# Sicco123/YieldFactorModels.jl

Hardware: AMD Instinct MI355X
Metric: Kalman loglik evals/sec (DNS, T=600, N=30) (higher is better)
Workload: dtype f64

## Files before the change

### yieldfactormodels.jl_amd/csrc/yfm_fixedz.hpp

```cpp
#pragma once
#pragma clang fp contract(off)
#include "yfm_device.hpp"

namespace yfm {

template <int M>
__device__ __forceinline__ double collapsed_cov(const double (&R)[M][M], const double (&Pm)[M][M], LDLT<M>& f,
                                                double (&Pf)[M][M]) {
  double S[M][M];
#pragma unroll
  for (int i = 0; i < M; ++i)
#pragma unroll
    for (int j = 0; j <= i; ++j) S[i][j] = Pm[i][j] + R[i][j];
  const double det = f.factor(S);
#pragma unroll
  for (int j = 0; j < M; ++j) {
    double xj[M];
#pragma unroll
    for (int i = 0; i < M; ++i) xj[i] = R[i][j];
    f.solve(xj);
#pragma unroll
    for (int i = 0; i <= j; ++i) {
      double s = 0.0;
#pragma unroll
// ... 433 lines not shown
    last_q = upd ? q : __builtin_nan("");
    if (acc) {
      if (STEADY && was_frozen) {
        count_frozen(det);
      } else {
        ld.mul(det);
        neg = neg || (det < 0.0);
      }
      sumq += last_q;
    }
  }

  __device__ __forceinline__ void record(int t, int b, int my_steps, int rec_len, double* __restrict__ rec_beta,
                                         double* __restrict__ rec_P) const {
    const int slot = t - max(0, my_steps - rec_len);
    if (t < my_steps && slot >= 0) {
      const size_t o = (size_t)b * (size_t)rec_len + slot;
#pragma unroll
      for (int i = 0; i < M; ++i) rec_beta[o * M + i] = beta[i];
      if (rec_P) {
#pragma unroll
        for (int j = 0; j < M; ++j)
#pragma unroll
          for (int i = 0; i < M; ++i) rec_P[o * M * M + j * M + i] = Pm[i][j];
      }
    }
  }

  __device__ __forceinline__ double loglik(int nobs, unsigned int* __restrict__ flags) const {
    double ll;
    if (!init_ok) {
      ll = __builtin_nan("");
      atomicAdd(&flags[0], 1u);
    } else {
      const int nterms = max(nobs - 2, 0);
      if (nterms == 0) {
        ll = 0.0;
      } else {
        const double per_term = (double)(N - M) * log(sigma2) + logdetG + (double)N * kLog2Pi;
        double lf = 0.0;
        if constexpr (STEADY) lf = fzlog + (nfz == 0 ? 0.0 : (double)nfz * log(fabs(fzdet)));
        ll = -0.5 * ((double)nterms * per_term + (ld.log_value() + lf) + sumq);
      }
      const bool fneg = STEADY && nfz != 0 && fzdet < 0.0;
      if (neg || fneg || !isfinite(ll)) {
        ll = -__builtin_inf();
        atomicAdd(&flags[1], 1u);
      }
    }
    return ll;
  }
};

}
```

### yieldfactormodels.jl_amd/csrc/yfm_internal.hpp

```cpp
#pragma once
#include "yfm_flags.hpp"
#include <hip/hip_runtime.h>

#include "../../include/yfm.h"

namespace yfm {

struct DevBuf {
  void* p = nullptr;
  size_t cap = 0;
  DevBuf() = default;
  DevBuf(const DevBuf&) = delete;
  DevBuf& operator=(const DevBuf&) = delete;
  ~DevBuf() {
    if (p) (void)hipFree(p);
  }
  hipError_t ensure(size_t bytes) {
    if (bytes <= cap) return hipSuccess;
    if (p) (void)hipFree(p);
    p = nullptr;
    cap = 0;
    hipError_t e = hipMalloc(&p, bytes);
    if (e == hipSuccess) cap = bytes;
    return e;
  }
};

struct LaunchArgs {
  const double* theta;
  int P, B, space;
  const double* panel;
  const double* raw;
  int T, N, np, ldp;
  const double* mats;
  const int* T_use;
  double* out;
  unsigned int* flags;
  unsigned int* flags_next = nullptr;
  double* rec_beta;
  double* rec_P;
  double* scratch;
  int horizon = 0;
  int rec_len = 0;
  int* defer_list = nullptr;
  int* defer_count = nullptr;
  hipStream_t stream;
};

int fixedz_np_for(int N);
hipError_t launch_fixedz(int kind, const LaunchArgs& a);
bool dns_split_supported(int np);
hipError_t launch_dns_split(const LaunchArgs& a);
size_t fixedz_scratch_bytes(int kind, int B);
int group_max_n(int kind);
int group_lanes_for(int kind, int N);
hipError_t launch_fixedz_group(int kind, const LaunchArgs& a);
size_t fixedz_dd_scratch_bytes(int kind, int B);
hipError_t launch_fixedz_dd(int kind, const LaunchArgs& a, double* rec);
int grad_max_n();
hipError_t launch_dns_grad(const LaunchArgs& a, const double* ll, double* grad_out);
int tvl_lanes_for(int B, int N, int share = 1);
int tvl_max_n();
size_t tvl_scratch_bytes(int B);
constexpr int kTvlGaps = 8;
constexpr int kTvlPowGaps = 16;
struct TvlGaps {
  int K = 0;
  bool exact = false;
  const double* d = nullptr;
  const int* idx = nullptr;
  int Kp = 0;
  double step = 0.0;
  const double* e = nullptr;
  const int* pidx = nullptr;
};
hipError_t launch_tvl(const LaunchArgs& a, const TvlGaps& g, int lanes);
constexpr int kRecSigma = 0, kRecDelta = 1, kRecPhi = 5, kRecQ = 21, kRecBeta = 31, kRecP = 35, kRecOk = 45;
constexpr int kRecLen = 48;
size_t tvl_dd_scratch_bytes(int B);
size_t tvl_dd_colsum_bytes(int T);
int tvl_dd_lanes_for(int B, int N, int want, int share = 1);
hipError_t launch_tvl_dd_colsum(const double* Y, int N, int T, double* colsum, hipStream_t s);
hipError_t launch_tvl_dd_init(const LaunchArgs& a, double* rec_dd);
hipError_t launch_tvl_dd(const LaunchArgs& a, const double* rec_dd, const double* colsum, const TvlGaps& g, int lanes);
struct PredictArgs {
  int kind, M, L, N, P, B, T;
  int ncol;
  int horizon;
  const double* theta;
  const double* mats;
  const int* T_use;
  const double* rec;
  int rec_len;
  const unsigned char* init_bad;
  double* preds;
  double* factors;
  double* states;
  double* load1;
  double* load2;
  hipStream_t stream;
};
hipError_t launch_init_bad(const double* ll, int B, unsigned char* bad, hipStream_t s);
hipError_t launch_predict_emit(const PredictArgs& a);
hipError_t launch_forecast_emit(const PredictArgs& a);
hipError_t launch_loss_array(const PredictArgs& a, const double* Y, int T1, int passes, unsigned int* flags);
// ... 12 lines not shown
```

### yieldfactormodels.jl_amd/csrc/yfm_kernels.hip

```cpp
#include "yfm_fixedz.hpp"

namespace yfm {

constexpr int kBlock = 256;
constexpr int kTC = 64;
constexpr bool kMfma4 = true;
constexpr bool kZBasis = true;

__global__ void prep_panel_kernel(const double* __restrict__ Y, int N, int T, int np, int ldp,
                                  double* __restrict__ out) {
  const int t = blockIdx.x * blockDim.x + threadIdx.x;
  if (t >= T) return;
  const double* y = Y + (size_t)t * N;
  double* o = out + (size_t)t * ldp;
  double s1 = 0.0, yy = 0.0;
  bool nan = false;
  for (int i = 0; i < N; ++i) {
    const double v = y[i];
    nan = nan || (v != v);
    s1 += v;
    yy = fma(v, v, yy);
  }
  const double ybar = s1 / (double)N;
  double tt = 0.0;
// ... 140 lines not shown
    }
    const double piv = col[k];
    ok = ok && (piv != 0.0);
    const double rp = 1.0 / piv;
#pragma unroll
    for (int i = k + 1; i < S; ++i) {
      const double l = col[i] * rp;
#pragma unroll
      for (int s = sk; s < NS; ++s) a[s][i] = fma(-l, a[s][k], a[s][i]);
    }
  }
  double x[S];
#pragma unroll
  for (int k = S - 1; k >= 0; --k) {
    const double rp = role_bcast_from<R>(k % R, 1.0 / a[k / R][k]);
    double s = role_bcast_from<R>(S % R, a[S / R][k]);
#pragma unroll
    for (int j = k + 1; j < S; ++j) s = role_bcast_from<R>(j % R, fma(-a[j / R][k], x[j], s));
    x[k] = s * rp;
  }
  if (role != 0) return;
  int q = 0;
#pragma unroll
  for (int i = 0; i < M; ++i) rec[(size_t)(q++) * B + b] = beta[i];
#pragma unroll
  for (int r = 0; r < S; ++r) rec[(size_t)(q++) * B + b] = x[r];
  rec[(size_t)q * B + b] = ok ? 1.0 : 0.0;
}


template <int NP, int NZ>
__device__ __forceinline__ void dot_zt(const double* __restrict__ col, const double (&Zc)[NZ][NP], double (&zt)[NZ]) {
  double a[NZ][2];
#pragma unroll
  for (int cz = 0; cz < NZ; ++cz) {
    a[cz][0] = 0.0;
    a[cz][1] = 0.0;
  }
#pragma unroll
  for (int i = 0; i < NP; i += 2) {
    const double2 y2 = *reinterpret_cast<const double2*>(col + i);
#pragma unroll
    for (int cz = 0; cz < NZ; ++cz) {
      a[cz][0] = fma(Zc[cz][i], y2.x, a[cz][0]);
      a[cz][1] = fma(Zc[cz][i + 1], y2.y, a[cz][1]);
    }
  }
#pragma unroll
  for (int cz = 0; cz < NZ; ++cz) zt[cz] = a[cz][0] + a[cz][1];
}

typedef double yfm_double4 __attribute__((ext_vector_type(4)));

template <int NP, int M, int LEAD, bool RECORD, bool STEADY_ = false, bool SPLIT_FORM = false>
__global__ __launch_bounds__(kBlock, 1) void fixedz_loglik_kernel(
    const double* __restrict__ theta, int P, int B, int space, const double* __restrict__ panel, int T, int N,
    const double* __restrict__ mats, const int* __restrict__ T_use, double* __restrict__ out,
    unsigned int* __restrict__ flags, double* __restrict__ rec_beta, double* __restrict__ rec_P, int horizon,
    int rec_len, int* __restrict__ defer_list, int* __restrict__ defer_count, const double* __restrict__ init_rec,
    unsigned int* __restrict__ flags_next, int steady) {
  constexpr int LDP = NP + 4;
  constexpr int TC = (M == 3) ? kTC : 32;
  constexpr bool USE_MFMA_ = (M - 1 == 2 || M - 1 == 4) && (NP <= 32);
  constexpr bool STEADY = STEADY_ && !RECORD && (M == 3 || M == 5) && USE_MFMA_;
  constexpr bool SPLIT_INIT = (M == 5);
  constexpr int CH = TC * LDP;
  constexpr int PER = (CH + kBlock - 1) / kBlock;
  constexpr int NZ = M - 1;
  constexpr bool USE_MFMA = (NZ == 2 || NZ == 4) && (NP <= 32);
  constexpr int NK = (NP + 3) / 4;
  constexpr int NRT = 64 * NZ / 16;
  constexpr int RGN = 4;
  constexpr int RGN4 = (NZ == 2) ? NRT : 8;
  constexpr int TB = 16;
  constexpr bool ZB = USE_MFMA && kMfma4 && kZBasis && LEAD == 2;
  constexpr int RPC = ZB ? LEAD : NZ;
  constexpr int NRTA = 64 * RPC / 16;
  constexpr int SS = 64 * NZ + 2;
  constexpr int SCR = USE_MFMA ? ((TB * SS > 32 * RPC * (4 * NK + 1)) ? TB * SS : 32 * RPC * (4 * NK + 1)) : 2;
  static_assert(NZ == 2 * LEAD, "loading columns come in (S, C) pairs per gamma");
  static_assert(NP % 2 == 0, "double2 panel reads");
  static_assert(TC % TB == 0, "MFMA blocks tile the panel chunk");
  __shared__ __attribute__((aligned(16))) double sh[2][CH];
  __shared__ __attribute__((aligned(16))) double scratch[kBlock / 64][SCR];
  __shared__ int s_nobs_max;
  __shared__ double s_rm[ZB ? NP : 1];

  if (flags_next && blockIdx.x == 0 && threadIdx.x < kFlagsPerBank) flags_next[threadIdx.x] = 0u;
  const int tid = threadIdx.x;
  const int lane = tid & 63;
  const int wave = tid >> 6;
  const int b = blockIdx.x * kBlock + tid;
  const bool live = b < B;
  const int bb = live ? b : (B - 1);
  const int nobs = T_use ? T_use[bb] : T;

  auto load_into = [&](double* dst, int c) {
    const size_t base = (size_t)c * CH;
    const size_t lim = (size_t)T * LDP;
#pragma unroll
    for (int r = 0; r < PER; ++r) {
      const int e = r * kBlock + tid;
      const size_t g = base + e;
      dst[r] = (e < CH && g < lim) ? panel[g] : 0.0;
    }
  };
  auto store_from = [&](const double* src, double* buf) {
#pragma unroll
    for (int r = 0; r < PER; ++r) {
      const int e = r * kBlock + tid;
      if (e < CH) buf[e] = src[r];
    }
  };
  constexpr bool EARLY = M == 3 && NP <= 32;
  double pre0[EARLY ? PER : 1], pre1[EARLY ? PER : 1];
  if constexpr (EARLY) {
    load_into(pre0, 0);
    load_into(pre1, 1);
  }

  if (tid == 0) s_nobs_max = 0;
  if constexpr (ZB) {
    for (int i = tid; i < NP; i += kBlock) s_rm[i] = (i < N) ? 1.0 / mats[i] : 0.0;
// ... 12 lines not shown
      const double* src = theta + (size_t)w0 * kP;
      double* thl = scratch[wave];
      double v[kP];
#pragma unroll
      for (int r = 0; r < kP; ++r) {
        const int e = r * 64 + lane;
        v[r] = (e < n) ? src[e] : 0.0;
      }
#pragma unroll
      for (int r = 0; r < kP; ++r) thl[r * 64 + lane] = v[r];
      __builtin_amdgcn_s_waitcnt(0xc07f);
      __builtin_amdgcn_wave_barrier();
      th_row = thl + (bb - w0) * kP;
    }
  }
  Params<M, LEAD> p;
  decode_params<M, LEAD>(th_row, space, p);
  __builtin_amdgcn_s_waitcnt(0xc07f);
  __builtin_amdgcn_wave_barrier();

  double Zc[NZ][NP];
#pragma unroll
  for (int l = 0; l < LEAD; ++l) {
    const double lam = 1e-2 + exp(p.gam[l]);
#pragma unroll
    for (int i = 0; i < NP; ++i) {
      const double tau = lam * mats[max(min(i, N - 1), 0)];
      const double z = exp(-tau);
      const double s = (1.0 - z) / tau;
      Zc[2 * l][i] = (i < N) ? s : 0.0;
      Zc[2 * l + 1][i] = (i < N) ? s - z : 0.0;
    }
  }
  double G[M][M];
  G[0][0] = (double)N;
#pragma unroll
  for (int c = 0; c < NZ; ++c) {
    double s = 0.0;
#pragma unroll
    for (int i = 0; i < NP; ++i) s += Zc[c][i];
    G[0][c + 1] = s;
    G[c + 1][0] = s;
#pragma unroll
    for (int d = c; d < NZ; ++d) {
      double g = 0.0;
#pragma unroll
      for (int i = 0; i < NP; ++i) g = fma(Zc[c][i], Zc[d][i], g);
      G[c + 1][d + 1] = g;
      G[d + 1][c + 1] = g;
    }
  }

  constexpr bool SIGMA = USE_MFMA && !ZB && !(kMfma4 && NZ == 4);
  constexpr bool IL = SIGMA && NRT == 2 * RGN && NK == 2 * RGN;
  constexpr bool IL5 = ZB && NK == NRTA;
  auto sigma = [](int i) { return SIGMA ? 4 * (i & 3) + (i >> 2) : i; };
  double Af[USE_MFMA ? NRTA : 1][USE_MFMA ? NK : 1];
  double rlam[LEAD];
#pragma unroll
  for (int l = 0; l < LEAD; ++l) rlam[l] = 1.0 / (1e-2 + exp(p.gam[l]));
  if constexpr (USE_MFMA) {
    constexpr int ZS = 4 * NK + 1;
    constexpr int HT = NRTA / 2;
    static_assert(32 * RPC * ZS <= SCR, "staging fits the scratch");
    double* st = scratch[wave];
#pragma unroll
    for (int h = 0; h < 2; ++h) {
      if ((lane >> 5) == h) {
        const int cl = lane & 31;
        if constexpr (ZB) {
#pragma unroll
          for (int l = 0; l < LEAD; ++l) {
            const double lam = 1e-2 + exp(p.gam[l]);
#pragma unroll
            for (int m = 0; m < ZS; ++m) {
              const double e = 1.0 - exp(-(lam * mats[max(min(m, N - 1), 0)]));
              st[(cl * RPC + l) * ZS + m] = (m < N) ? e : 0.0;
            }
          }
        } else {
#pragma unroll
          for (int c = 0; c < NZ; ++c)
#pragma unroll
            for (int m = 0; m < ZS; ++m) st[(cl * NZ + c) * ZS + m] = (m < NP) ? Zc[c][m] : 0.0;
        }
      }
      __builtin_amdgcn_s_waitcnt(0xc07f);
      __builtin_amdgcn_wave_barrier();
#pragma unroll
      for (int r = h * HT; r < (h + 1) * HT; ++r) {
        const int pr = 16 * r + sigma(lane & 15) - h * 32 * RPC;
#pragma unroll
        for (int kk = 0; kk < NK; ++kk) Af[r][kk] = st[pr * ZS + 4 * kk + (lane >> 4)];
      }
      __builtin_amdgcn_s_waitcnt(0xc07f);
      __builtin_amdgcn_wave_barrier();
    }
  }

  FixedZFilter<M, LEAD, RECORD, STEADY, SPLIT_FORM> f;
  f.p = p;
  f.steady_ok = steady != 0;
  f.setup(G, N, !SPLIT_INIT);
  if constexpr (SPLIT_INIT) {
    int q = 0;
#pragma unroll
    for (int i = 0; i < M; ++i) f.beta[i] = init_rec[(size_t)(q++) * B + bb];
#pragma unroll
    for (int i = 0; i < M; ++i)
#pragma unroll
      for (int j = i; j < M; ++j) {
        const double v = init_rec[(size_t)(q++) * B + bb];
        f.Pm[i][j] = v;
        f.Pm[j][i] = v;
      }
    f.init_ok = init_rec[(size_t)q * B + bb] != 0.0;
  }
  const bool defer = live && !f.collapsed;
  if (defer) defer_list[atomicAdd(defer_count, 1)] = b;

  int wmin = live ? my_data : 0x7fffffff;
#pragma unroll
  for (int off = 32; off >= 1; off >>= 1) wmin = min(wmin, __shfl_xor(wmin, off));
  const int wave_min_data = __builtin_amdgcn_readfirstlane(wmin);
  const bool wave_all_collapsed = true;

  __syncthreads();
  const int nsteps = max(s_nobs_max, 0);

  double pre[PER];
  auto load_chunk = [&](int c) { load_into(pre, c); };
  auto store_chunk = [&](double* buf) { store_from(pre, buf); };
  if (nsteps > 0) {
    if constexpr (EARLY) {
      store_from(pre0, sh[0]);
      store_from(pre1, sh[1]);
    } else {
// ... 106 lines not shown
            const int m = 4 * kk + (lane >> 4);
            const double y = (m < NP) ? cb[(2 * sp + ((lane & 3) >> 1)) * LDP + m] : 0.0;
            bv[kk] = (lane & 1) ? y * s_rm[m < NP ? m : 0] : y;
          }
#pragma unroll
          for (int r0 = 0; r0 < NRTA; r0 += NRTA) {
            double acc[NRTA];
#pragma unroll
            for (int r = 0; r < NRTA; ++r) acc[r] = 0.0;
#pragma unroll
            for (int kk = 0; kk < NK; ++kk)
#pragma unroll
              for (int r = 0; r < NRTA; ++r)
                acc[r] = __builtin_amdgcn_mfma_f64_4x4x4f64(Af[r][kk], bv[kk], acc[r], 0, 0, 0);
#pragma unroll
            for (int r = 0; r < NRTA; ++r)
              scr[(2 * sp + ((lane & 3) >> 1)) * SS + 2 * (16 * r + 4 * ((lane >> 2) & 3) + (lane >> 4)) + (lane & 1)] =
                  acc[r];
          }
        }
      } else if constexpr (kMfma4 && NZ == 4) {
#pragma unroll
        for (int s = 0; s < TB / 4; ++s) {
          double bv[NK];
#pragma unroll
          for (int kk = 0; kk < NK; ++kk) {
            const int m = 4 * kk + (lane >> 4);
            bv[kk] = (m < NP) ? cb[(4 * s + (lane & 3)) * LDP + m] : 0.0;
          }
#pragma unroll
          for (int r0 = 0; r0 < NRT; r0 += RGN4) {
            double acc[RGN4];
#pragma unroll
            for (int r = 0; r < RGN4; ++r) acc[r] = 0.0;
#pragma unroll
            for (int kk = 0; kk < NK; ++kk)
#pragma unroll
              for (int r = 0; r < RGN4; ++r)
                acc[r] = __builtin_amdgcn_mfma_f64_4x4x4f64(Af[r0 + r][kk], bv[kk], acc[r], 0, 0, 0);
#pragma unroll
            for (int r = 0; r < RGN4; ++r)
              scr[(4 * s + (lane & 3)) * SS + 16 * (r0 + r) + 4 * ((lane >> 2) & 3) + (lane >> 4)] = acc[r];
          }
        }
      } else {
        double bvk[NK];
#pragma unroll
        for (int kk = 0; kk < NK; ++kk) {
          const int m = 4 * kk + (lane >> 4);
          bvk[kk] = (m < NP) ? cb[(lane & 15) * LDP + m] : 0.0;
        }
        if constexpr (IL) {
          constexpr int H = RGN / 2;
          yfm_double4 a1[RGN], a2[H], a3[H];
#pragma unroll
          for (int r = 0; r < RGN; ++r) a1[r] = yfm_double4{0.0, 0.0, 0.0, 0.0};
#pragma unroll
          for (int r = 0; r < H; ++r) a2[r] = a3[r] = yfm_double4{0.0, 0.0, 0.0, 0.0};
#pragma unroll
          for (int kk = 0; kk < NK; ++kk)
#pragma unroll
            for (int r = 0; r < RGN; ++r)
              a1[r] = __builtin_amdgcn_mfma_f64_16x16x4f64(Af[r][kk], bvk[kk], a1[r], 0, 0, 0);
#pragma unroll
          for (int kk = 0; kk < NK; ++kk) {
#pragma unroll
            for (int r = 0; r < H; ++r)
              a2[r] = __builtin_amdgcn_mfma_f64_16x16x4f64(Af[RGN + r][kk], bvk[kk], a2[r], 0, 0, 0);
            const int r1 = kk >> 1, h = kk & 1;
            double* d = scr + (lane & 15) * SS + 16 * r1 + 4 * (lane >> 4) + 2 * h;
            *reinterpret_cast<double2*>(d) = make_double2(a1[r1][2 * h], a1[r1][2 * h + 1]);
          }
#pragma unroll
          for (int kk = 0; kk < NK; ++kk) {
#pragma unroll
            for (int r = 0; r < H; ++r)
              a3[r] = __builtin_amdgcn_mfma_f64_16x16x4f64(Af[RGN + H + r][kk], bvk[kk], a3[r], 0, 0, 0);
            if (kk & 1) {
              const int r2 = kk >> 2, h = (kk >> 1) & 1;
              double* d = scr + (lane & 15) * SS + 16 * (RGN + r2) + 4 * (lane >> 4) + 2 * h;
              *reinterpret_cast<double2*>(d) = make_double2(a2[r2][2 * h], a2[r2][2 * h + 1]);
            }
          }
          __builtin_amdgcn_sched_group_barrier(0x008, RGN * NK, 0);
#pragma unroll
          for (int kk = 0; kk < NK; ++kk) {
            __builtin_amdgcn_sched_group_barrier(0x008, H, 0);
            __builtin_amdgcn_sched_group_barrier(0x200, 1, 0);
          }
#pragma unroll
          for (int kk = 0; kk < NK; ++kk) {
            __builtin_amdgcn_sched_group_barrier(0x008, H, 0);
            if (kk & 1) __builtin_amdgcn_sched_group_barrier(0x200, 1, 0);
          }
#pragma unroll
          for (int r = 0; r < H; ++r) store_tile(scr, RGN + H + r, a3[r]);
        } else {
#pragma unroll
        for (int r0 = 0; r0 < NRT; r0 += RGN) {
          yfm_double4 acc[RGN];
#pragma unroll
          for (int r = 0; r < RGN; ++r) acc[r] = yfm_double4{0.0, 0.0, 0.0, 0.0};
#pragma unroll
          for (int kk = 0; kk < NK; ++kk)
#pragma unroll
            for (int r = 0; r < RGN; ++r)
              acc[r] = __builtin_amdgcn_mfma_f64_16x16x4f64(Af[r0 + r][kk], bvk[kk], acc[r], 0, 0, 0);
#pragma unroll
          for (int r = 0; r < RGN; ++r) store_tile(scr, r0 + r, acc[r]);
        }
        }
      }
      __builtin_amdgcn_s_waitcnt(0xc07f);
      __builtin_amdgcn_wave_barrier();
      const int tend = min(TB, nsteps - t0);
      bool blk_steady = false;
      if constexpr (STEADY) {
        if (__all(f.wave_frozen) && t0 >= 1 && t0 + tend <= wave_min_data) {
          const bool col_nan = (lane < tend) && (col_flag != 0.0);
          blk_steady = !__any(col_nan);
        }
      }
      auto read_z = [&](int tt, double (&z)[NZ]) {
        const double* sp = scr + tt * SS + NZ * lane;
#pragma unroll
        for (int j = 0; j < NZ; j += 2) {
          const double2 v = *reinterpret_cast<const double2*>(sp + j);
          if constexpr (ZB) {
            z[j] = rlam[j / 2] * v.y;
            z[j + 1] = z[j] + v.x;
          } else {
            z[j] = v.x;
            z[j + 1] = v.y;
          }
        }
      };
      double zc[NZ];
      read_z(0, zc);
      double2 yb = *reinterpret_cast<const double2*>(cb + NP);
      double2 meta = *reinterpret_cast<const double2*>(cb + NP + 2);
      double zn[NZ];
      double2 ybn, metan;
      auto half = [&](int tt, const double (&zc_)[NZ], double2 yb_, double2 meta_, double (&zn_)[NZ], double2& ybn_,
                      double2& metan_) {
        const int t = t0 + tt;
        const int tn = min(tt + 1, TB - 1);
        read_z(tn, zn_);
        ybn_ = *reinterpret_cast<const double2*>(cb + tn * LDP + NP);
        metan_ = *reinterpret_cast<const double2*>(cb + tn * LDP + NP + 2);
        do_step(t, zc_, yb_, meta_);
        record(t);
        if ((t + 1) % TC == 0) rot_t = t;
      };
      auto shalf = [&](int tt, const double (&zc_)[NZ], double2 yb_, double (&zn_)[NZ], double2& ybn_) {
        const int tn = min(tt + 1, TB - 1);
        read_z(tn, zn_);
        ybn_ = *reinterpret_cast<const double2*>(cb + tn * LDP + NP);
        f.steady_step(zc_, yb_);
        if ((t0 + tt + 1) % TC == 0) rot_t = t0 + tt;
      };
      if constexpr (STEADY) {
        if (blk_steady) {
          if (tend == TB) {
            double zq[2][NZ];
            double2 ybq[2];
#pragma unroll
            for (int j = 0; j < NZ; ++j) zq[0][j] = zc[j];
            ybq[0] = yb;
#pragma unroll
            for (int u = 0; u < TB; ++u) {
              const int cur = u & 1, nx = cur ^ 1;
              const int tn = min(u + 1, TB - 1);
              read_z(tn, zq[nx]);
              ybq[nx] = *reinterpret_cast<const double2*>(cb + tn * LDP + NP);
              f.steady_step(zq[cur], ybq[cur]);
            }
            rot_t = ((t0 + TB) % TC == 0) ? t0 + TB - 1 : -1;
          } else {
            int tt = 0;
            for (; tt + 1 < tend; tt += 2) {
              shalf(tt, zc, yb, zn, ybn);
              shalf(tt + 1, zn, ybn, zc, yb);
            }
            if (tt < tend) shalf(tt, zc, yb, zn, ybn);
          }
          steady_steps += tend;
          f.count_steady(tend);
        }
      }
      if (!blk_steady) {
        int tt = 0;
        bool rest_steady = false;
        for (; tt + 1 < tend; tt += 2) {
          half(tt, zc, yb, meta, zn, ybn, metan);
          half(tt + 1, zn, ybn, metan, zc, yb, meta);
          if constexpr (STEADY) {
            if (tt == TB / 2 - 2) f.prepare_bound();
            {
              const int r0 = tt + 2;
              if (r0 >= TB / 2 && r0 < tend && t0 + tend <= wave_min_data) {
                const bool nan_rest = (lane >= r0) && (lane < tend) && (col_flag != 0.0);
                if (!__any(nan_rest)) {
                  f.wave_freeze(live && !defer && f.init_ok && t0 + tend <= my_steps);
                  if (f.wave_frozen) {
                    rest_steady = true;
                    tt = r0;
                    break;
                  }
                }
              }
            }
          }
        }
        if constexpr (STEADY) {
          if (rest_steady) {
            const int n = tend - tt;
            for (; tt + 1 < tend; tt += 2) {
              shalf(tt, zc, yb, zn, ybn);
              shalf(tt + 1, zn, ybn, zc, yb);
            }
            if (tt < tend) shalf(tt, zc, yb, zn, ybn);
            steady_steps += n;
            f.count_steady(n);
          }
        }
        if (!rest_steady) {
          if (tt < tend) half(tt, zc, yb, meta, zn, ybn, metan);
          if constexpr (STEADY) f.wave_freeze(live && !defer && f.init_ok && t0 + tend <= my_steps);
        }
      }
      __builtin_amdgcn_s_waitcnt(0xc07f);
      __builtin_amdgcn_wave_barrier();
    }
    if (rot_t >= 0) rotate(rot_t);
    if constexpr (STEADY) {
      if (lane == 0 && steady_steps) atomicAdd(&flags[4], steady_steps);
    }
  } else {
    double zc[NZ];
    double2 yb_c = make_double2(0.0, 0.0), meta_c = make_double2(0.0, 0.0);
    if (nsteps > 0) {
      const double* c0 = col_of(0);
      dot_zt<NP, NZ>(c0, Zc, zc);
      yb_c = *reinterpret_cast<const double2*>(c0 + NP);
      meta_c = *reinterpret_cast<const double2*>(c0 + NP + 2);
    }
    double zn[NZ];
    double2 yb_n, meta_n;
    auto half = [&](int t, const double (&zc_)[NZ], double2 yb_, double2 meta_, double (&zn_)[NZ], double2& ybn_,
                    double2& metan_) {
      const double* cn = col_of(t + 1);
      dot_zt<NP, NZ>(cn, Zc, zn_);
      ybn_ = *reinterpret_cast<const double2*>(cn + NP);
      metan_ = *reinterpret_cast<const double2*>(cn + NP + 2);
      do_step(t, zc_, yb_, meta_);
      record(t);
      rotate(t);
    };
    int t = 0;
    for (; t + 1 < nsteps; t += 2) {
      half(t, zc, yb_c, meta_c, zn, yb_n, meta_n);
      half(t + 1, zn, yb_n, meta_n, zc, yb_c, meta_c);
    }
    if (t < nsteps) half(t, zc, yb_c, meta_c, zn, yb_n, meta_n);
  }

  if (!live || defer) return;
  const double ll = f.loglik(nobs, flags);
  out[b] = ll;
}

}

#include "yfm_internal.hpp"

#include <cstdlib>

namespace yfm {

static int steady_enabled() {
  const char* e = std::getenv("YFM_DNS_STEADY");
  return (e && e[0] == '0') ? 0 : 1;
}

static int gns5_steady_enabled() {
  const char* e = std::getenv("YFM_GNS5_STEADY");
  return (e && e[0] == '1') ? 1 : 0;
}

static int split_form_enabled() {
  const char* e = std::getenv("YFM_FZ_SPLIT_FORM");
  return (e && e[0] == '1') ? 1 : 0;
}

static int gns5_init_lanes() {
  const char* e = std::getenv("YFM_GNS5_INIT_LANES");
  return (e && e[0] == '1' && e[1] == 0) ? 1 : 2;
}

template <int NP, int M, int LEAD>
static hipError_t launch_fixedz_np(const LaunchArgs& a) {
  const int grid = (a.B + kBlock - 1) / kBlock;
  if constexpr (M == 5) {
    if (!a.scratch) return hipErrorInvalidValue;
    const int ir = gns5_init_lanes();
    if (ir == 1) {
      hipLaunchKernelGGL((fixedz_init_kernel<M, LEAD>), dim3(grid), dim3(kBlock), 0, a.stream, a.theta, a.P, a.B,
                         a.space, a.scratch, a.flags_next);
    } else {
      const int gi = (int)(((size_t)a.B * 2 + kBlock - 1) / kBlock);
      hipLaunchKernelGGL((fixedz_init_coop_kernel<M, LEAD, 2>), dim3(gi), dim3(kBlock), 0, a.stream, a.theta, a.P, a.B,
                         a.space, a.scratch, a.flags_next);
    }
  }
  if (a.rec_beta) {
    hipLaunchKernelGGL((fixedz_loglik_kernel<NP, M, LEAD, true>), dim3(grid), dim3(kBlock), 0, a.stream, a.theta, a.P,
                       a.B, a.space, a.panel, a.T, a.N, a.mats, a.T_use, a.out, a.flags, a.rec_beta, a.rec_P,
                       a.horizon, a.rec_len, a.defer_list, a.defer_count, a.scratch, M == 5 ? nullptr : a.flags_next, 0);
  } else {
    constexpr bool kSteady = (M == 3 || M == 5) && (NP <= 32);
    constexpr int kSteadyMinT = 80;
    const bool on = steady_enabled() && a.T >= kSteadyMinT && (M != 5 || gns5_steady_enabled());
    auto* k = (kSteady && on) ? &fixedz_loglik_kernel<NP, M, LEAD, false, kSteady>
                              : &fixedz_loglik_kernel<NP, M, LEAD, false, false>;
    constexpr bool kSplitForm = (M == 5) && (NP == 30 || NP == 48);
    if constexpr (kSplitForm) {
      if (split_form_enabled()) k = &fixedz_loglik_kernel<NP, M, LEAD, false, false, true>;
    }
    hipLaunchKernelGGL(k, dim3(grid), dim3(kBlock), 0, a.stream, a.theta, a.P, a.B, a.space, a.panel, a.T, a.N,
                       a.mats, a.T_use, a.out, a.flags, nullptr, nullptr, 0, 0, a.defer_list, a.defer_count,
                       a.scratch, M == 5 ? nullptr : a.flags_next, 1);
  }
  return hipGetLastError();
}

size_t fixedz_scratch_bytes(int kind, int B) {
  return kind == 2 ? sizeof(double) * (size_t)fz_rec_len<5>() * (size_t)(B > 0 ? B : 1) : 0;
}

int fixedz_np_for(int N) {
  if (N <= 8) return 8;
  if (N <= 16) return 16;
  if (N <= 24) return 24;
  if (N <= 30) return 30;
  if (N <= 32) return 32;
  if (N <= 48) return 48;
  if (N <= 64) return 64;
  return -1;
}

hipError_t launch_fixedz(int kind, const LaunchArgs& a) {
  if (kind == 0 && dns_split_supported(a.np)) {
    const char* e = std::getenv("YFM_DNS_SPLIT");
    if (e && e[0] == '1') return launch_dns_split(a);
  }
  if (kind == 0) {
    switch (a.np) {
      case 8: return launch_fixedz_np<8, 3, 1>(a);
      case 16: return launch_fixedz_np<16, 3, 1>(a);
      case 24: return launch_fixedz_np<24, 3, 1>(a);
      case 30: return launch_fixedz_np<30, 3, 1>(a);
      case 32: return launch_fixedz_np<32, 3, 1>(a);
      case 48: return launch_fixedz_np<48, 3, 1>(a);
      case 64: return launch_fixedz_np<64, 3, 1>(a);
    }
  } else if (kind == 2) {
    switch (a.np) {
      case 8: return launch_fixedz_np<8, 5, 2>(a);
      case 16: return launch_fixedz_np<16, 5, 2>(a);
      case 24: return launch_fixedz_np<24, 5, 2>(a);
      case 30: return launch_fixedz_np<30, 5, 2>(a);
      case 32: return launch_fixedz_np<32, 5, 2>(a);
      case 48: return launch_fixedz_np<48, 5, 2>(a);
      case 64: return launch_fixedz_np<64, 5, 2>(a);
    }
  }
  return hipErrorInvalidValue;
}

hipError_t launch_prep_panel(const double* Y, int N, int T, int np, int ldp, double* out, hipStream_t s) {
  hipLaunchKernelGGL(prep_panel_kernel, dim3((T + 63) / 64), dim3(64), 0, s, Y, N, T, np, ldp, out);
// ... 5 lines not shown
```

### yieldfactormodels.jl_amd/csrc/yfm_split.hip

```cpp
#include "yfm_fixedz.hpp"
#include "yfm_internal.hpp"

#include <cstdlib>
#include <type_traits>

namespace yfm {

namespace {

constexpr int kSplitBlock = 512;
constexpr int kSplitPairs = 4;
constexpr int kSTC = 32;
constexpr int kSTB = 16;
constexpr int kRec = 13;

}

template <int NP, bool RECORD>
__global__ __launch_bounds__(kSplitBlock, 1) void dns_split_kernel(
    const double* __restrict__ theta, int P, int B, int space, const double* __restrict__ panel, int T, int N,
    const double* __restrict__ mats, const int* __restrict__ T_use, double* __restrict__ out,
    unsigned int* __restrict__ flags, double* __restrict__ rec_beta, double* __restrict__ rec_P, int horizon,
    int rec_len, int* __restrict__ defer_list, int* __restrict__ defer_count, int interleave,
    unsigned int* __restrict__ flags_next) {
  constexpr int M = 3, LEAD = 1, NZ = 2;
  if (flags_next && blockIdx.x == 0 && threadIdx.x < kFlagsPerBank) flags_next[threadIdx.x] = 0u;
  constexpr int LDP = NP + 4;
  constexpr int CH = kSTC * LDP;
  constexpr int PER = (CH + kSplitBlock - 1) / kSplitBlock;
  constexpr int NK = (NP + 3) / 4;
  constexpr int NRT = 64 * NZ / 16;
  constexpr int SS = 64 * NZ + 2;
  constexpr int SCR = kSTB * SS;
  static_assert(NP <= 32 && NP % 2 == 0, "MFMA fragments and double2 panel reads");
  __shared__ __attribute__((aligned(16))) double sh[2][CH];
  __shared__ __attribute__((aligned(16))) double scratch[kSplitPairs][SCR];
  __shared__ double ring[2][kSplitPairs][kRec][64];
  __shared__ int s_nobs_max;

  const int tid = threadIdx.x;
  const int lane = tid & 63;
  const int wave = tid >> 6;
  const bool cov = interleave ? !(wave & 1) : wave < kSplitPairs;
  const int pair = interleave ? (wave >> 1) : (wave & (kSplitPairs - 1));
  const int b = blockIdx.x * (kSplitPairs * 64) + pair * 64 + lane;
  const bool live = b < B;
  const int bb = live ? b : (B - 1);
  const int nobs = T_use ? T_use[bb] : T;

  if (tid == 0) s_nobs_max = 0;
  __syncthreads();
  const int my_steps = horizon > 0 ? nobs + horizon : nobs - 1;
  const int my_data = horizon > 0 ? nobs : nobs - 1;
  atomicMax(&s_nobs_max, live ? my_steps : 0);

  auto role = [&](auto is_cov) {
    constexpr bool COV = decltype(is_cov)::value;
  FixedZFilter<M, LEAD, RECORD> f;
  decode_params<M, LEAD>(theta + (size_t)bb * P, space, f.p);
  const double lam = 1e-2 + exp(f.p.gam[0]);
  auto loading = [&](int i, double& s, double& c) {
    if (i < N) {
      const double tau = lam * mats[i];
      const double z = exp(-tau);
      s = (1.0 - z) / tau;
      c = s - z;
    } else {
      s = 0.0;
      c = 0.0;
    }
  };
  double G[M][M];
  double gs[NZ] = {0.0, 0.0}, gg[3] = {0.0, 0.0, 0.0};
  auto acc_gram = [&](double s, double c) {
    gs[0] += s;
    gs[1] += c;
    gg[0] = fma(s, s, gg[0]);
    gg[1] = fma(s, c, gg[1]);
    gg[2] = fma(c, c, gg[2]);
  };
#pragma unroll
  for (int i = 0; i < NP; ++i) {
    double zs, zc;
    loading(i, zs, zc);
    acc_gram(zs, zc);
  }
  G[0][0] = (double)N;
  G[0][1] = G[1][0] = gs[0];
  G[0][2] = G[2][0] = gs[1];
  G[1][1] = gg[0];
  G[1][2] = G[2][1] = gg[1];
  G[2][2] = gg[2];
  f.setup(G, N, true);
  const bool defer = live && !f.collapsed;
  if constexpr (!COV) {
    if (defer) defer_list[atomicAdd(defer_count, 1)] = b;
  }
  double Af[COV ? 1 : NRT][COV ? 1 : NK];
  if constexpr (!COV) {
    constexpr int ZS = 4 * NK + 1;
    constexpr int QT = NRT / 4;
    static_assert(16 * NZ * ZS <= SCR, "staging fits the scratch");
    double* st = scratch[pair];
#pragma unroll
    for (int qu = 0; qu < 4; ++qu) {
      if ((lane >> 4) == qu) {
        const int cl = lane & 15;
#pragma unroll
        for (int m = 0; m < ZS; ++m) {
          double zs, zc;
          loading(m < NP ? m : NP, zs, zc);
          st[(cl * NZ + 0) * ZS + m] = zs;
          st[(cl * NZ + 1) * ZS + m] = zc;
        }
      }
      __builtin_amdgcn_s_waitcnt(0xc07f);
      __builtin_amdgcn_wave_barrier();
#pragma unroll
      for (int r = qu * QT; r < (qu + 1) * QT; ++r) {
        const int pr = 16 * r + (lane & 15) - qu * 16 * NZ;
#pragma unroll
        for (int kk = 0; kk < NK; ++kk) Af[r][kk] = st[pr * ZS + 4 * kk + (lane >> 4)];
      }
      __builtin_amdgcn_s_waitcnt(0xc07f);
      __builtin_amdgcn_wave_barrier();
    }
  }

  int wmin = live ? my_data : 0x7fffffff;
#pragma unroll
  for (int off = 32; off >= 1; off >>= 1) wmin = min(wmin, __shfl_xor(wmin, off));
  const int wave_min_data = __builtin_amdgcn_readfirstlane(wmin);

  __syncthreads();
  const int nsteps = max(s_nobs_max, 0);

  double pre[PER];
  auto load_chunk = [&](int c) {
    const size_t base = (size_t)c * CH;
    const size_t lim = (size_t)T * LDP;
#pragma unroll
    for (int r = 0; r < PER; ++r) {
      const int e = r * kSplitBlock + tid;
      const size_t g = base + e;
      pre[r] = (e < CH && g < lim) ? panel[g] : 0.0;
    }
  };
  auto store_chunk = [&](double* buf) {
#pragma unroll
    for (int r = 0; r < PER; ++r) {
      const int e = r * kSplitBlock + tid;
      if (e < CH) buf[e] = pre[r];
    }
  };
  if (nsteps > 0) {
    load_chunk(0);
    store_chunk(sh[0]);
    load_chunk(1);
    store_chunk(sh[1]);
    __syncthreads();
    load_chunk(2);
  }
  auto col_of = [&](int t) -> const double* { return sh[(t / kSTC) & 1] + (t % kSTC) * LDP; };
  auto lds_barrier = [] {
// ... 45 lines not shown
#pragma unroll
            for (int j = i; j < M; ++j) Pf[i][j] = f.Pm[i][j];
          propagate_cov_f<M>(phi, f.p.Q, Pf, f.Pm);
        }
        if constexpr (RECORD) {
          const int rs = t - max(0, my_steps - rec_len);
          if (rec_P && live && !defer && act && rs >= 0) {
            const size_t o = (size_t)b * (size_t)rec_len + rs;
#pragma unroll
            for (int j = 0; j < M; ++j)
#pragma unroll
              for (int i = 0; i < M; ++i) rec_P[o * M * M + j * M + i] = f.Pm[i][j];
          }
        }
      }
      end_iteration(k);
    }
  } else {
  double* scr = scratch[pair];
  for (int k = 0; k <= nsteps; ++k) {
    if (k >= 1) {
      const int t = k - 1;
      const int tt = t % kSTB;
      if (tt == 0) {
        const double* cb = col_of(t);
        double bvk[NK];
#pragma unroll
        for (int kk = 0; kk < NK; ++kk) {
          const int m = 4 * kk + (lane >> 4);
          bvk[kk] = (m < NP) ? cb[(lane & 15) * LDP + m] : 0.0;
        }
        typedef double d4 __attribute__((ext_vector_type(4)));
        constexpr int RG = NRT / 4;
#pragma unroll
        for (int r0 = 0; r0 < NRT; r0 += RG) {
          d4 acc[RG];
#pragma unroll
          for (int r = 0; r < RG; ++r) acc[r] = d4{0.0, 0.0, 0.0, 0.0};
#pragma unroll
          for (int kk = 0; kk < NK; ++kk)
#pragma unroll
            for (int r = 0; r < RG; ++r)
              acc[r] = __builtin_amdgcn_mfma_f64_16x16x4f64(Af[r0 + r][kk], bvk[kk], acc[r], 0, 0, 0);
#pragma unroll
          for (int r = 0; r < RG; ++r)
#pragma unroll
            for (int q4 = 0; q4 < 4; ++q4) scr[(lane & 15) * SS + 16 * (r0 + r) + (lane >> 4) + 4 * q4] = acc[r][q4];
        }
        __builtin_amdgcn_s_waitcnt(0xc07f);
        __builtin_amdgcn_wave_barrier();
      }
      const double* cb = col_of(t);
      const double2 z2 = *reinterpret_cast<const double2*>(scr + tt * SS + NZ * lane);
      const double zc[NZ] = {z2.x, z2.y};
      const double2 yb = *reinterpret_cast<const double2*>(cb + NP);
      const double2 meta = *reinterpret_cast<const double2*>(cb + NP + 2);
      const bool fast = (t >= 1) && (meta.x == 0.0) && (t < wave_min_data);
      const bool act = t < my_steps;
      if (fast || (act && meta.x == 0.0 && t < my_data)) {
        const double* slot = &ring[t & 1][pair][0][lane];
        LDLT<M> fl;
        fl.L[1][0] = slot[0 * 64];
        fl.L[2][0] = slot[1 * 64];
        fl.L[2][1] = slot[2 * 64];
        fl.rd[0] = slot[3 * 64];
        fl.rd[1] = slot[4 * 64];
        fl.rd[2] = slot[5 * 64];
        double Pm[M][M];
        Pm[0][0] = slot[6 * 64];
        Pm[0][1] = Pm[1][0] = slot[7 * 64];
        Pm[0][2] = Pm[2][0] = slot[8 * 64];
        Pm[1][1] = slot[9 * 64];
        Pm[1][2] = Pm[2][1] = slot[10 * 64];
        Pm[2][2] = slot[11 * 64];
        const double det = slot[12 * 64];
        double bf[M], q;
        collapsed_mean<M>(zc, yb.x, yb.y, f.R, f.rsig2, f.beta, Pm, fl, bf, q);
        if (fast) {
          if (!RECORD || det != 0.0) propagate_mean_f<M>(phi, f.p.delta, bf, f.beta);
          f.last_det = det;
          f.last_q = q;
          f.ld.mul(det);
          f.sumq += q;
          f.neg = f.neg || (det < 0.0);
        } else {
          const bool upd = det != 0.0;
          if (upd) propagate_mean_f<M>(phi, f.p.delta, bf, f.beta);
          f.last_det = det;
          f.last_q = upd ? q : __builtin_nan("");
          if (t >= 1) {
            f.ld.mul(det);
            f.sumq += f.last_q;
            f.neg = f.neg || (det < 0.0);
          }
        }
      } else if (act) {
        double bf[M];
#pragma unroll
        for (int i = 0; i < M; ++i) bf[i] = f.beta[i];
        propagate_mean_f<M>(phi, f.p.delta, bf, f.beta);
        if (t >= 1) {
          f.ld.mul(f.last_det);
          f.sumq += f.last_q;
          f.neg = f.neg || (f.last_det < 0.0);
        }
      }
      if constexpr (RECORD) {
        const int rs = t - max(0, my_steps - rec_len);
        if (live && !defer && act && rs >= 0) {
          const size_t o = (size_t)b * (size_t)rec_len + rs;
#pragma unroll
          for (int i = 0; i < M; ++i) rec_beta[o * M + i] = f.beta[i];
        }
      }
      if (tt == kSTB - 1) {
        __builtin_amdgcn_s_waitcnt(0xc07f);
        __builtin_amdgcn_wave_barrier();
      }
    }
    end_iteration(k);
  }

  if (!live || defer) return;
  out[b] = f.loglik(nobs, flags);
  }

  };
  if (cov)
    role(std::true_type{});
  else
    role(std::false_type{});
}

namespace {

template <int NP>
hipError_t launch_split_np(const LaunchArgs& a) {
  const int interleave = 0;
  const int grid = (a.B + kSplitPairs * 64 - 1) / (kSplitPairs * 64);
  if (a.rec_beta) {
    hipLaunchKernelGGL((dns_split_kernel<NP, true>), dim3(grid), dim3(kSplitBlock), 0, a.stream, a.theta, a.P, a.B,
                       a.space, a.panel, a.T, a.N, a.mats, a.T_use, a.out, a.flags, a.rec_beta, a.rec_P, a.horizon,
                       a.rec_len, a.defer_list, a.defer_count, interleave, a.flags_next);
  } else {
    hipLaunchKernelGGL((dns_split_kernel<NP, false>), dim3(grid), dim3(kSplitBlock), 0, a.stream, a.theta, a.P, a.B,
                       a.space, a.panel, a.T, a.N, a.mats, a.T_use, a.out, a.flags, nullptr, nullptr, 0, 0,
                       a.defer_list, a.defer_count, interleave, a.flags_next);
  }
  return hipGetLastError();
}

}

bool dns_split_supported(int np) { return np == 8 || np == 16 || np == 24 || np == 30 || np == 32; }

hipError_t launch_dns_split(const LaunchArgs& a) {
  switch (a.np) {
    case 8: return launch_split_np<8>(a);
    case 16: return launch_split_np<16>(a);
    case 24: return launch_split_np<24>(a);
    case 30: return launch_split_np<30>(a);
    case 32: return launch_split_np<32>(a);
  }
  return hipErrorInvalidValue;
}

}
```

Baseline: 375.7 million.

## Trim MFMA K-dimension for N=30 DNS by folding loading column into difference form

For NP=30, M=3, the loading matrix is rewritten as differences against the last observed column, so the projection needs only 28 K-slots (7 MFMA k-steps instead of 8). The leftover column at slot 28 is added back per step with an FMA using the raw panel value. Interleaved scheduling barriers and tile stores are generalized to odd NK. This cuts MFMA work in the projection at the cost of an extra load and FMA per step, and it relies on the panel's padding and column layout being arranged so that the difference form reproduces the original sums.

```diff
diff --git a/yieldfactormodels.jl_amd/csrc/yfm_fixedz.hpp b/yieldfactormodels.jl_amd/csrc/yfm_fixedz.hpp
--- a/yieldfactormodels.jl_amd/csrc/yfm_fixedz.hpp
+++ b/yieldfactormodels.jl_amd/csrc/yfm_fixedz.hpp
@@ -509,4 +509,19 @@
   }
 };
 
-}
+constexpr int kTrimNP = 30;
+constexpr int kTrimSlot = 28;
+constexpr bool ktrim_applies(int NP, int M) { return NP == kTrimNP && M == 3; }
+constexpr int ktrim_nk(int NP, bool trim) { return trim ? (kTrimSlot / 4) : (NP + 3) / 4; }
+
+__device__ __forceinline__ double ktrim_diff(double z, double z_last, int i, int N) {
+  return (i < N - 1) ? z - z_last : 0.0;
+}
+
+template <int NZ>
+__device__ __forceinline__ void ktrim_leftover(const double (&zd)[NZ], const double (&zx)[NZ + 1], double (&z)[NZ]) {
+#pragma unroll
+  for (int c = 0; c < NZ; ++c) z[c] = fma(zd[c], zx[NZ], zx[c]);
+}
+
+}
diff --git a/yieldfactormodels.jl_amd/csrc/yfm_internal.hpp b/yieldfactormodels.jl_amd/csrc/yfm_internal.hpp
--- a/yieldfactormodels.jl_amd/csrc/yfm_internal.hpp
+++ b/yieldfactormodels.jl_amd/csrc/yfm_internal.hpp
@@ -51,6 +51,7 @@
 hipError_t launch_fixedz(int kind, const LaunchArgs& a);
 bool dns_split_supported(int np);
 hipError_t launch_dns_split(const LaunchArgs& a);
+int ktrim_enabled();
 size_t fixedz_scratch_bytes(int kind, int B);
 int group_max_n(int kind);
 int group_lanes_for(int kind, int N);
diff --git a/yieldfactormodels.jl_amd/csrc/yfm_kernels.hip b/yieldfactormodels.jl_amd/csrc/yfm_kernels.hip
--- a/yieldfactormodels.jl_amd/csrc/yfm_kernels.hip
+++ b/yieldfactormodels.jl_amd/csrc/yfm_kernels.hip
@@ -216,8 +216,8 @@
 
 typedef double yfm_double4 __attribute__((ext_vector_type(4)));
 
-template <int NP, int M, int LEAD, bool RECORD, bool STEADY_ = false, bool SPLIT_FORM = false>
-__global__ __launch_bounds__(kBlock, 1) void fixedz_loglik_kernel(
+template <int NP, int M, int LEAD, bool RECORD, bool STEADY_, bool SPLIT_FORM, bool KTRIM_>
+__device__ __forceinline__ void fixedz_loglik_body(
     const double* __restrict__ theta, int P, int B, int space, const double* __restrict__ panel, int T, int N,
     const double* __restrict__ mats, const int* __restrict__ T_use, double* __restrict__ out,
     unsigned int* __restrict__ flags, double* __restrict__ rec_beta, double* __restrict__ rec_P, int horizon,
@@ -232,7 +232,8 @@
   constexpr int PER = (CH + kBlock - 1) / kBlock;
   constexpr int NZ = M - 1;
   constexpr bool USE_MFMA = (NZ == 2 || NZ == 4) && (NP <= 32);
-  constexpr int NK = (NP + 3) / 4;
+  constexpr bool KTRIM = KTRIM_ && USE_MFMA && ktrim_applies(NP, M);
+  constexpr int NK = ktrim_nk(NP, KTRIM);
   constexpr int NRT = 64 * NZ / 16;
   constexpr int RGN = 4;
   constexpr int RGN4 = (NZ == 2) ? NRT : 8;
@@ -351,10 +352,21 @@
   }
 
   constexpr bool SIGMA = USE_MFMA && !ZB && !(kMfma4 && NZ == 4);
-  constexpr bool IL = SIGMA && NRT == 2 * RGN && NK == 2 * RGN;
+  constexpr bool IL = SIGMA && NRT == 2 * RGN && (NK == 2 * RGN || NK == 2 * RGN - 1);
   constexpr bool IL5 = ZB && NK == NRTA;
   auto sigma = [](int i) { return SIGMA ? 4 * (i & 3) + (i >> 2) : i; };
   double Af[USE_MFMA ? NRTA : 1][USE_MFMA ? NK : 1];
+  double z_last[KTRIM ? NZ : 1], zd28[KTRIM ? NZ : 1];
+  if constexpr (KTRIM) {
+#pragma unroll
+    for (int c = 0; c < NZ; ++c) {
+      double zl = 0.0;
+#pragma unroll
+      for (int i = 0; i < NP; ++i) zl = (i == N - 1) ? Zc[c][i] : zl;
+      z_last[c] = zl;
+      zd28[c] = ktrim_diff(Zc[c][kTrimSlot], zl, kTrimSlot, N);
+    }
+  }
   double rlam[LEAD];
 #pragma unroll
   for (int l = 0; l < LEAD; ++l) rlam[l] = 1.0 / (1e-2 + exp(p.gam[l]));
@@ -381,7 +393,12 @@
 #pragma unroll
           for (int c = 0; c < NZ; ++c)
 #pragma unroll
-            for (int m = 0; m < ZS; ++m) st[(cl * NZ + c) * ZS + m] = (m < NP) ? Zc[c][m] : 0.0;
+            for (int m = 0; m < ZS; ++m) {
+              if constexpr (KTRIM)
+                st[(cl * NZ + c) * ZS + m] = ktrim_diff(Zc[c][m], z_last[c], m, N);
+              else
+                st[(cl * NZ + c) * ZS + m] = (m < NP) ? Zc[c][m] : 0.0;
+            }
         }
       }
       __builtin_amdgcn_s_waitcnt(0xc07f);
@@ -594,6 +611,9 @@
         }
         if constexpr (IL) {
           constexpr int H = RGN / 2;
+          constexpr int NS1 = 2 * RGN, NS2 = 2 * H;
+          auto last1 = [](int kk) { return kk == NK - 1 ? NS1 : kk + 1; };
+          auto at2 = [](int s) { return 2 * s + 1 < NK - 1 ? 2 * s + 1 : NK - 1; };
           yfm_double4 a1[RGN], a2[H], a3[H];
 #pragma unroll
           for (int r = 0; r < RGN; ++r) a1[r] = yfm_double4{0.0, 0.0, 0.0, 0.0};
@@ -609,31 +629,40 @@
 #pragma unroll
             for (int r = 0; r < H; ++r)
               a2[r] = __builtin_amdgcn_mfma_f64_16x16x4f64(Af[RGN + r][kk], bvk[kk], a2[r], 0, 0, 0);
-            const int r1 = kk >> 1, h = kk & 1;
-            double* d = scr + (lane & 15) * SS + 16 * r1 + 4 * (lane >> 4) + 2 * h;
-            *reinterpret_cast<double2*>(d) = make_double2(a1[r1][2 * h], a1[r1][2 * h + 1]);
+#pragma unroll
+            for (int s = kk; s < last1(kk); ++s) {
+              const int r1 = s >> 1, h = s & 1;
+              double* d = scr + (lane & 15) * SS + 16 * r1 + 4 * (lane >> 4) + 2 * h;
+              *reinterpret_cast<double2*>(d) = make_double2(a1[r1][2 * h], a1[r1][2 * h + 1]);
+            }
           }
 #pragma unroll
           for (int kk = 0; kk < NK; ++kk) {
 #pragma unroll
             for (int r = 0; r < H; ++r)
               a3[r] = __builtin_amdgcn_mfma_f64_16x16x4f64(Af[RGN + H + r][kk], bvk[kk], a3[r], 0, 0, 0);
-            if (kk & 1) {
-              const int r2 = kk >> 2, h = (kk >> 1) & 1;
-              double* d = scr + (lane & 15) * SS + 16 * (RGN + r2) + 4 * (lane >> 4) + 2 * h;
-              *reinterpret_cast<double2*>(d) = make_double2(a2[r2][2 * h], a2[r2][2 * h + 1]);
+#pragma unroll
+            for (int s = 0; s < NS2; ++s) {
+              if (at2(s) == kk) {
+                const int r2 = s >> 1, h = s & 1;
+                double* d = scr + (lane & 15) * SS + 16 * (RGN + r2) + 4 * (lane >> 4) + 2 * h;
+                *reinterpret_cast<double2*>(d) = make_double2(a2[r2][2 * h], a2[r2][2 * h + 1]);
+              }
             }
           }
           __builtin_amdgcn_sched_group_barrier(0x008, RGN * NK, 0);
 #pragma unroll
           for (int kk = 0; kk < NK; ++kk) {
             __builtin_amdgcn_sched_group_barrier(0x008, H, 0);
-            __builtin_amdgcn_sched_group_barrier(0x200, 1, 0);
+#pragma unroll
+            for (int s = kk; s < last1(kk); ++s) __builtin_amdgcn_sched_group_barrier(0x200, 1, 0);
           }
 #pragma unroll
           for (int kk = 0; kk < NK; ++kk) {
             __builtin_amdgcn_sched_group_barrier(0x008, H, 0);
-            if (kk & 1) __builtin_amdgcn_sched_group_barrier(0x200, 1, 0);
+#pragma unroll
+            for (int s = 0; s < NS2; ++s)
+              if (at2(s) == kk) __builtin_amdgcn_sched_group_barrier(0x200, 1, 0);
           }
 #pragma unroll
           for (int r = 0; r < H; ++r) store_tile(scr, RGN + H + r, a3[r]);
@@ -663,7 +692,17 @@
           blk_steady = !__any(col_nan);
         }
       }
-      auto read_z = [&](int tt, double (&z)[NZ]) {
+      constexpr int NZX = NZ + (KTRIM ? 1 : 0);
+      auto z_of = [&](const double (&zx)[NZX], double (&z)[NZ]) {
+        if constexpr (KTRIM) {
+          ktrim_leftover<NZ>(zd28, zx, z);
+        } else {
+#pragma unroll
+          for (int j = 0; j < NZ; ++j) z[j] = zx[j];
+        }
+      };
+      auto read_z = [&](int tt, double (&z)[NZX]) {
+        if constexpr (KTRIM) z[NZ] = reinterpret_cast<const double2*>(cb + tt * LDP + kTrimSlot)->x;
         const double* sp = scr + tt * SS + NZ * lane;
 #pragma unroll
         for (int j = 0; j < NZ; j += 2) {
@@ -677,37 +716,41 @@
           }
         }
       };
-      double zc[NZ];
+      double zc[NZX];
       read_z(0, zc);
       double2 yb = *reinterpret_cast<const double2*>(cb + NP);
       double2 meta = *reinterpret_cast<const double2*>(cb + NP + 2);
-      double zn[NZ];
+      double zn[NZX];
       double2 ybn, metan;
-      auto half = [&](int tt, const double (&zc_)[NZ], double2 yb_, double2 meta_, double (&zn_)[NZ], double2& ybn_,
+      auto half = [&](int tt, const double (&zc_)[NZX], double2 yb_, double2 meta_, double (&zn_)[NZX], double2& ybn_,
                       double2& metan_) {
         const int t = t0 + tt;
         const int tn = min(tt + 1, TB - 1);
         read_z(tn, zn_);
         ybn_ = *reinterpret_cast<const double2*>(cb + tn * LDP + NP);
         metan_ = *reinterpret_cast<const double2*>(cb + tn * LDP + NP + 2);
-        do_step(t, zc_, yb_, meta_);
+        double z[NZ];
+        z_of(zc_, z);
+        do_step(t, z, yb_, meta_);
         record(t);
         if ((t + 1) % TC == 0) rot_t = t;
       };
-      auto shalf = [&](int tt, const double (&zc_)[NZ], double2 yb_, double (&zn_)[NZ], double2& ybn_) {
+      auto shalf = [&](int tt, const double (&zc_)[NZX], double2 yb_, double (&zn_)[NZX], double2& ybn_) {
         const int tn = min(tt + 1, TB - 1);
         read_z(tn, zn_);
         ybn_ = *reinterpret_cast<const double2*>(cb + tn * LDP + NP);
-        f.steady_step(zc_, yb_);
+        double z[NZ];
+        z_of(zc_, z);
+        f.steady_step(z, yb_);
         if ((t0 + tt + 1) % TC == 0) rot_t = t0 + tt;
       };
       if constexpr (STEADY) {
         if (blk_steady) {
           if (tend == TB) {
-            double zq[2][NZ];
+            double zq[2][NZX];
             double2 ybq[2];
 #pragma unroll
-            for (int j = 0; j < NZ; ++j) zq[0][j] = zc[j];
+            for (int j = 0; j < NZX; ++j) zq[0][j] = zc[j];
             ybq[0] = yb;
 #pragma unroll
             for (int u = 0; u < TB; ++u) {
@@ -715,7 +758,9 @@
               const int tn = min(u + 1, TB - 1);
               read_z(tn, zq[nx]);
               ybq[nx] = *reinterpret_cast<const double2*>(cb + tn * LDP + NP);
-              f.steady_step(zq[cur], ybq[cur]);
+              double z[NZ];
+              z_of(zq[cur], z);
+              f.steady_step(z, ybq[cur]);
             }
             rot_t = ((t0 + TB) % TC == 0) ? t0 + TB - 1 : -1;
           } else {
@@ -812,6 +857,30 @@
   out[b] = ll;
 }
 
+template <int NP, int M, int LEAD, bool RECORD, bool STEADY_ = false, bool SPLIT_FORM = false>
+__global__ __launch_bounds__(kBlock, 1) void fixedz_loglik_kernel(
+    const double* __restrict__ theta, int P, int B, int space, const double* __restrict__ panel, int T, int N,
+    const double* __restrict__ mats, const int* __restrict__ T_use, double* __restrict__ out,
+    unsigned int* __restrict__ flags, double* __restrict__ rec_beta, double* __restrict__ rec_P, int horizon,
+    int rec_len, int* __restrict__ defer_list, int* __restrict__ defer_count, const double* __restrict__ init_rec,
+    unsigned int* __restrict__ flags_next, int steady) {
+  fixedz_loglik_body<NP, M, LEAD, RECORD, STEADY_, SPLIT_FORM, true>(
+      theta, P, B, space, panel, T, N, mats, T_use, out, flags, rec_beta, rec_P, horizon, rec_len, defer_list,
+      defer_count, init_rec, flags_next, steady);
+}
+
+template <int NP, int M, int LEAD, bool RECORD, bool STEADY_, bool SPLIT_FORM, bool KTRIM_>
+__global__ __launch_bounds__(kBlock, 1) void fixedz_loglik_kernel(
+    const double* __restrict__ theta, int P, int B, int space, const double* __restrict__ panel, int T, int N,
+    const double* __restrict__ mats, const int* __restrict__ T_use, double* __restrict__ out,
+    unsigned int* __restrict__ flags, double* __restrict__ rec_beta, double* __restrict__ rec_P, int horizon,
+    int rec_len, int* __restrict__ defer_list, int* __restrict__ defer_count, const double* __restrict__ init_rec,
+    unsigned int* __restrict__ flags_next, int steady) {
+  fixedz_loglik_body<NP, M, LEAD, RECORD, STEADY_, SPLIT_FORM, KTRIM_>(
+      theta, P, B, space, panel, T, N, mats, T_use, out, flags, rec_beta, rec_P, horizon, rec_len, defer_list,
+      defer_count, init_rec, flags_next, steady);
+}
+
 }
 
 #include "yfm_internal.hpp"
@@ -822,6 +891,11 @@
 
 static int steady_enabled() {
   const char* e = std::getenv("YFM_DNS_STEADY");
+  return (e && e[0] == '0') ? 0 : 1;
+}
+
+int ktrim_enabled() {
+  const char* e = std::getenv("YFM_DNS_KTRIM");
   return (e && e[0] == '0') ? 0 : 1;
 }
 
@@ -855,8 +929,15 @@
                          a.space, a.scratch, a.flags_next);
     }
   }
+  constexpr bool kTrimmable = ktrim_applies(NP, M) && (NP <= 32);
+  bool untrimmed = false;
+  if constexpr (kTrimmable) untrimmed = !ktrim_enabled();
   if (a.rec_beta) {
-    hipLaunchKernelGGL((fixedz_loglik_kernel<NP, M, LEAD, true>), dim3(grid), dim3(kBlock), 0, a.stream, a.theta, a.P,
+    auto* k = &fixedz_loglik_kernel<NP, M, LEAD, true, false, false>;
+    if constexpr (kTrimmable) {
+      if (untrimmed) k = &fixedz_loglik_kernel<NP, M, LEAD, true, false, false, false>;
+    }
+    hipLaunchKernelGGL(k, dim3(grid), dim3(kBlock), 0, a.stream, a.theta, a.P,
                        a.B, a.space, a.panel, a.T, a.N, a.mats, a.T_use, a.out, a.flags, a.rec_beta, a.rec_P,
                        a.horizon, a.rec_len, a.defer_list, a.defer_count, a.scratch, M == 5 ? nullptr : a.flags_next, 0);
   } else {
@@ -869,6 +950,11 @@
     if constexpr (kSplitForm) {
       if (split_form_enabled()) k = &fixedz_loglik_kernel<NP, M, LEAD, false, false, true>;
     }
+    if constexpr (kTrimmable) {
+      if (untrimmed)
+        k = (kSteady && on) ? &fixedz_loglik_kernel<NP, M, LEAD, false, kSteady, false, false>
+                            : &fixedz_loglik_kernel<NP, M, LEAD, false, false, false, false>;
+    }
     hipLaunchKernelGGL(k, dim3(grid), dim3(kBlock), 0, a.stream, a.theta, a.P, a.B, a.space, a.panel, a.T, a.N,
                        a.mats, a.T_use, a.out, a.flags, nullptr, nullptr, 0, 0, a.defer_list, a.defer_count,
                        a.scratch, M == 5 ? nullptr : a.flags_next, 1);
diff --git a/yieldfactormodels.jl_amd/csrc/yfm_split.hip b/yieldfactormodels.jl_amd/csrc/yfm_split.hip
--- a/yieldfactormodels.jl_amd/csrc/yfm_split.hip
+++ b/yieldfactormodels.jl_amd/csrc/yfm_split.hip
@@ -16,7 +16,7 @@
 
 }
 
-template <int NP, bool RECORD>
+template <int NP, bool RECORD, bool KTRIM_>
 __global__ __launch_bounds__(kSplitBlock, 1) void dns_split_kernel(
     const double* __restrict__ theta, int P, int B, int space, const double* __restrict__ panel, int T, int N,
     const double* __restrict__ mats, const int* __restrict__ T_use, double* __restrict__ out,
@@ -28,7 +28,8 @@
   constexpr int LDP = NP + 4;
   constexpr int CH = kSTC * LDP;
   constexpr int PER = (CH + kSplitBlock - 1) / kSplitBlock;
-  constexpr int NK = (NP + 3) / 4;
+  constexpr bool KTRIM = KTRIM_ && ktrim_applies(NP, M);
+  constexpr int NK = ktrim_nk(NP, KTRIM);
   constexpr int NRT = 64 * NZ / 16;
   constexpr int SS = 64 * NZ + 2;
   constexpr int SCR = kSTB * SS;
@@ -97,7 +98,16 @@
     if (defer) defer_list[atomicAdd(defer_count, 1)] = b;
   }
   double Af[COV ? 1 : NRT][COV ? 1 : NK];
+  double zd28[NZ] = {0.0, 0.0};
   if constexpr (!COV) {
+    double zl_s = 0.0, zl_c = 0.0;
+    if constexpr (KTRIM) {
+      loading(max(N - 1, 0), zl_s, zl_c);
+      double zs, zc;
+      loading(kTrimSlot, zs, zc);
+      zd28[0] = ktrim_diff(zs, zl_s, kTrimSlot, N);
+      zd28[1] = ktrim_diff(zc, zl_c, kTrimSlot, N);
+    }
     constexpr int ZS = 4 * NK + 1;
     constexpr int QT = NRT / 4;
     static_assert(16 * NZ * ZS <= SCR, "staging fits the scratch");
@@ -110,6 +120,10 @@
         for (int m = 0; m < ZS; ++m) {
           double zs, zc;
           loading(m < NP ? m : NP, zs, zc);
+          if constexpr (KTRIM) {
+            zs = ktrim_diff(zs, zl_s, m, N);
+            zc = ktrim_diff(zc, zl_c, m, N);
+          }
           st[(cl * NZ + 0) * ZS + m] = zs;
           st[(cl * NZ + 1) * ZS + m] = zc;
         }
@@ -261,7 +275,11 @@
       }
       const double* cb = col_of(t);
       const double2 z2 = *reinterpret_cast<const double2*>(scr + tt * SS + NZ * lane);
-      const double zc[NZ] = {z2.x, z2.y};
+      double zc[NZ] = {z2.x, z2.y};
+      if constexpr (KTRIM) {
+        const double zx[NZ + 1] = {z2.x, z2.y, reinterpret_cast<const double2*>(cb + kTrimSlot)->x};
+        ktrim_leftover<NZ>(zd28, zx, zc);
+      }
       const double2 yb = *reinterpret_cast<const double2*>(cb + NP);
       const double2 meta = *reinterpret_cast<const double2*>(cb + NP + 2);
       const bool fast = (t >= 1) && (meta.x == 0.0) && (t < wave_min_data);
@@ -343,16 +361,16 @@
 
 namespace {
 
-template <int NP>
+template <int NP, bool KTRIM = true>
 hipError_t launch_split_np(const LaunchArgs& a) {
   const int interleave = 0;
   const int grid = (a.B + kSplitPairs * 64 - 1) / (kSplitPairs * 64);
   if (a.rec_beta) {
-    hipLaunchKernelGGL((dns_split_kernel<NP, true>), dim3(grid), dim3(kSplitBlock), 0, a.stream, a.theta, a.P, a.B,
+    hipLaunchKernelGGL((dns_split_kernel<NP, true, KTRIM>), dim3(grid), dim3(kSplitBlock), 0, a.stream, a.theta, a.P, a.B,
                        a.space, a.panel, a.T, a.N, a.mats, a.T_use, a.out, a.flags, a.rec_beta, a.rec_P, a.horizon,
                        a.rec_len, a.defer_list, a.defer_count, interleave, a.flags_next);
   } else {
-    hipLaunchKernelGGL((dns_split_kernel<NP, false>), dim3(grid), dim3(kSplitBlock), 0, a.stream, a.theta, a.P, a.B,
+    hipLaunchKernelGGL((dns_split_kernel<NP, false, KTRIM>), dim3(grid), dim3(kSplitBlock), 0, a.stream, a.theta, a.P, a.B,
                        a.space, a.panel, a.T, a.N, a.mats, a.T_use, a.out, a.flags, nullptr, nullptr, 0, 0,
                        a.defer_list, a.defer_count, interleave, a.flags_next);
   }
@@ -368,7 +386,7 @@
     case 8: return launch_split_np<8>(a);
     case 16: return launch_split_np<16>(a);
     case 24: return launch_split_np<24>(a);
-    case 30: return launch_split_np<30>(a);
+    case 30: return ktrim_enabled() ? launch_split_np<30>(a) : launch_split_np<30, false>(a);
     case 32: return launch_split_np<32>(a);
   }
   return hipErrorInvalidValue;
```

New measurement: 385.2 million, median of 6. 2.5% higher.
